# icdm-adteam/MoCoPCI

Hardware: AMD Instinct MI355X
Metric: interpolated frames/sec (higher is better)
Workload: dtype f32 (fused MLP layers: fp32 products as 6 bf16-MFMA partials of an exact 3-way split, fp32 accumulate; index paths exact f32)

## Files before the change

mocopci_amd/csrc/fusion.hip:

```cpp
#include <stdlib.h>

#include "common.h"
#include "mfma_split.h"

namespace {

typedef float f32x16 __attribute__((ext_vector_type(16)));

constexpr int C1 = 64, C2 = 64, NB = 64;
constexpr int WAVES = 4;


__device__ __forceinline__ int chan_of(int r, int h) { return (r & 3) + 8 * (r >> 2) + 4 * h; }

__device__ __forceinline__ float wave_sum(float v) {
#pragma unroll
    for (int o = 32; o > 0; o >>= 1) v += __shfl_xor(v, o);
    return v;
}
__device__ __forceinline__ float wave_max(float v) {
#pragma unroll
    for (int o = 32; o > 0; o >>= 1) v = fmaxf(v, __shfl_xor(v, o));
    return v;
}

#ifdef MCP_AB
constexpr int OFF_W1 = 0, OFF_W2 = 256, OFF_W3 = OFF_W2 + 4096, OFF_B1 = OFF_W3 + 8192, OFF_B2 = OFF_B1 + 64,
              OFF_B3 = OFF_B2 + 64, LDS_FLOATS = OFF_B3 + 128;
__global__ __launch_bounds__(64 * WAVES, 2) void fusion_kernel(long long total, int n, const float *__restrict__ p1,
                                                            const float *__restrict__ p2, const int *__restrict__ idx, const int *__restrict__ idx2,
                                                            const float *__restrict__ w1, const float *__restrict__ b1,
                                                            const float *__restrict__ w2, const float *__restrict__ b2,
                                                            const float *__restrict__ w3, const float *__restrict__ b3,
                                                            float *__restrict__ out) {
    __shared__ __attribute__((aligned(16))) float lds[LDS_FLOATS];
    const int tid = threadIdx.x;
    for (int e = tid; e < 256; e += 64 * WAVES) {
        const int lane = e & 63, s = (e >> 6) & 1, t = e >> 7;
        lds[OFF_W1 + e] = w1[(32 * t + (lane & 31)) * 4 + 2 * s + (lane >> 5)];
    }
    for (int e = tid; e < 4096; e += 64 * WAVES) {
        const int j = e & 3, lane = (e >> 2) & 63, q = (e >> 8) & 7, t = e >> 11;
        const int s = 4 * q + j, tin = s >> 4, r = s & 15;
        lds[OFF_W2 + e] = w2[(32 * t + (lane & 31)) * C1 + 32 * tin + chan_of(r, lane >> 5)];
    }
    for (int e = tid; e < 8192; e += 64 * WAVES) {
        const int j = e & 3, lane = (e >> 2) & 63, q = (e >> 8) & 7, t = e >> 11;
        const int s = 4 * q + j, tin = s >> 4, r = s & 15;
        lds[OFF_W3 + e] = w3[(32 * t + (lane & 31)) * C2 + 32 * tin + chan_of(r, lane >> 5)];
    }
    for (int e = tid; e < 64; e += 64 * WAVES) {
        const int r = e & 15, h = (e >> 4) & 1, t = e >> 5;
        lds[OFF_B1 + e] = b1[32 * t + chan_of(r, h)];
        lds[OFF_B2 + e] = b2[32 * t + chan_of(r, h)];
    }
    for (int e = tid; e < 128; e += 64 * WAVES) {
        const int r = e & 15, h = (e >> 4) & 1, t = e >> 5;
        lds[OFF_B3 + e] = b3[32 * t + chan_of(r, h)];
    }
    __syncthreads();

    const int lane = tid & 63, wave = tid >> 6, h = lane >> 5, col = lane & 31;
    const float4 *w2q = reinterpret_cast<const float4 *>(lds + OFF_W2);
    const float4 *w3q = reinterpret_cast<const float4 *>(lds + OFF_W3);

    const McpUnits units = mcp_units_by_xcd(total, WAVES);
    for (long long p = units.first + wave; p < units.limit; p += units.stride) {
        const long long bb = mcp_div(p, n, mcp_fits32(total));
        const float cx = p1[p * 3 + 0], cy = p1[p * 3 + 1], cz = p1[p * 3 + 2];
        float score[2], nbx[2], nby[2], nbz[2];
#pragma unroll
        for (int ct = 0; ct < 2; ++ct) {
            const int id = idx2 ? (ct ? idx2 : idx)[p * 32 + col] : idx[p * NB + 32 * ct + col];
            const float *q = p2 + ((long long)bb * n + id) * 3;
            const float x = q[0], y = q[1], z = q[2];
            nbx[ct] = x; nby[ct] = y; nbz[ct] = z;
            const float rx = x - cx, ry = y - cy, rz = z - cz;
            const float dist = sqrtf((rx * rx + ry * ry) + rz * rz);
            const float in0 = h ? ry : rx, in1 = h ? dist : rz;
            f32x16 a1[2];
#pragma unroll
            for (int t = 0; t < 2; ++t) {
                f32x16 acc;
#pragma unroll
                for (int r = 0; r < 16; ++r) acc[r] = lds[OFF_B1 + (t * 2 + h) * 16 + r];
                acc = __builtin_amdgcn_mfma_f32_32x32x2f32(lds[OFF_W1 + (t * 2 + 0) * 64 + lane], in0, acc, 0, 0, 0);
                acc = __builtin_amdgcn_mfma_f32_32x32x2f32(lds[OFF_W1 + (t * 2 + 1) * 64 + lane], in1, acc, 0, 0, 0);
#pragma unroll
                for (int r = 0; r < 16; ++r) acc[r] = fmaxf(acc[r], 0.f);
                a1[t] = acc;
            }
            f32x16 a2[2];
#pragma unroll
            for (int t = 0; t < 2; ++t) {
                f32x16 acc;
#pragma unroll
                for (int r = 0; r < 16; ++r) acc[r] = lds[OFF_B2 + (t * 2 + h) * 16 + r];
#pragma unroll
                for (int q4 = 0; q4 < 8; ++q4) {
                    const float4 w = w2q[(t * 8 + q4) * 64 + lane];
                    const int tin = q4 >> 2, r0 = (q4 & 3) * 4;
                    acc = __builtin_amdgcn_mfma_f32_32x32x2f32(w.x, a1[tin][r0 + 0], acc, 0, 0, 0);
                    acc = __builtin_amdgcn_mfma_f32_32x32x2f32(w.y, a1[tin][r0 + 1], acc, 0, 0, 0);
                    acc = __builtin_amdgcn_mfma_f32_32x32x2f32(w.z, a1[tin][r0 + 2], acc, 0, 0, 0);
                    acc = __builtin_amdgcn_mfma_f32_32x32x2f32(w.w, a1[tin][r0 + 3], acc, 0, 0, 0);
                }
#pragma unroll
                for (int r = 0; r < 16; ++r) acc[r] = fmaxf(acc[r], 0.f);
                a2[t] = acc;
            }
            float m = 0.f;
#pragma unroll 1
            for (int t = 0; t < 4; ++t) {
                f32x16 acc;
#pragma unroll
                for (int r = 0; r < 16; ++r) acc[r] = lds[OFF_B3 + (t * 2 + h) * 16 + r];
#pragma unroll
                for (int q4 = 0; q4 < 8; ++q4) {
                    const float4 w = w3q[(t * 8 + q4) * 64 + lane];
                    const int tin = q4 >> 2, r0 = (q4 & 3) * 4;
                    acc = __builtin_amdgcn_mfma_f32_32x32x2f32(w.x, a2[tin][r0 + 0], acc, 0, 0, 0);
                    acc = __builtin_amdgcn_mfma_f32_32x32x2f32(w.y, a2[tin][r0 + 1], acc, 0, 0, 0);
                    acc = __builtin_amdgcn_mfma_f32_32x32x2f32(w.z, a2[tin][r0 + 2], acc, 0, 0, 0);
                    acc = __builtin_amdgcn_mfma_f32_32x32x2f32(w.w, a2[tin][r0 + 3], acc, 0, 0, 0);
                }
#pragma unroll
                for (int r = 0; r < 16; ++r) m = fmaxf(m, acc[r]);
            }
            score[ct] = fmaxf(m, __shfl_xor(m, 32));
        }
        const float mx = wave_max(fmaxf(score[0], score[1]));
        const float e0 = expf(score[0] - mx), e1 = expf(score[1] - mx);
        const float den = wave_sum(e0 + e1);
        const float sx = wave_sum(e0 * nbx[0] + e1 * nbx[1]);
        const float sy = wave_sum(e0 * nby[0] + e1 * nby[1]);
        const float sz = wave_sum(e0 * nbz[0] + e1 * nbz[1]);
        if (lane == 0) {
            out[p * 3 + 0] = sx / den;
            out[p * 3 + 1] = sy / den;
            out[p * 3 + 2] = sz / den;
        }
    }
}
#endif


constexpr int SP_W1 = 0, SP_B1 = 256, SP_B2 = SP_B1 + 64, SP_B3 = SP_B2 + 64, SP_F32_FLOATS = SP_B3 + 128;
constexpr int SP_W2_U4 = 2 * 4 * 3 * 64, SP_W3_U4 = 4 * 4 * 3 * 64;
constexpr size_t SP_LDS_BYTES = SP_F32_FLOATS * 4 + (size_t)(SP_W2_U4 + SP_W3_U4) * 16;

__global__ __launch_bounds__(64 * WAVES, 2) void fusion_split_kernel(long long total, int n, const float *__restrict__ p1,
                                                                  const float *__restrict__ p2, const int *__restrict__ idx, const int *__restrict__ idx2,
                                                                  const float *__restrict__ w1, const float *__restrict__ b1,
                                                                  const float *__restrict__ w2, const float *__restrict__ b2,
                                                                  const float *__restrict__ w3, const float *__restrict__ b3,
                                                                  float *__restrict__ out) {
    extern __shared__ __attribute__((aligned(16))) float lds[];
    uint4 *w2s = reinterpret_cast<uint4 *>(lds + SP_F32_FLOATS);
    uint4 *w3s = w2s + SP_W2_U4;
    const int tid = threadIdx.x;
    for (int e = tid; e < 256; e += 64 * WAVES) {
        const int lane = e & 63, s = (e >> 6) & 1, t = e >> 7;
        lds[SP_W1 + e] = w1[(32 * t + (lane & 31)) * 4 + 2 * s + (lane >> 5)];
    }
    mcp_split_weights(w2s, w2, C1, 2, tid, 64 * WAVES);
    mcp_split_weights(w3s, w3, C2, 4, tid, 64 * WAVES);
    for (int e = tid; e < 64; e += 64 * WAVES) {
        const int r = e & 15, h = (e >> 4) & 1, t = e >> 5;
        lds[SP_B1 + e] = b1[32 * t + chan_of(r, h)];
        lds[SP_B2 + e] = b2[32 * t + chan_of(r, h)];
    }
    for (int e = tid; e < 128; e += 64 * WAVES) {
        const int r = e & 15, h = (e >> 4) & 1, t = e >> 5;
        lds[SP_B3 + e] = b3[32 * t + chan_of(r, h)];
    }
    __syncthreads();

    const int lane = tid & 63, wave = tid >> 6, h = lane >> 5, col = lane & 31;
    const McpUnits units = mcp_units_by_xcd(total, WAVES);
    for (long long p = units.first + wave; p < units.limit; p += units.stride) {
        const long long bb = mcp_div(p, n, mcp_fits32(total));
        const float cx = p1[p * 3 + 0], cy = p1[p * 3 + 1], cz = p1[p * 3 + 2];
        float score[2], nbx[2], nby[2], nbz[2];
#pragma unroll
        for (int ct = 0; ct < 2; ++ct) {
            const int id = idx2 ? (ct ? idx2 : idx)[p * 32 + col] : idx[p * NB + 32 * ct + col];
            const float *q = p2 + ((long long)bb * n + id) * 3;
            const float x = q[0], y = q[1], z = q[2];
            nbx[ct] = x; nby[ct] = y; nbz[ct] = z;
            const float rx = x - cx, ry = y - cy, rz = z - cz;
            const float dist = sqrtf((rx * rx + ry * ry) + rz * rz);
            const float in0 = h ? ry : rx, in1 = h ? dist : rz;
            McpSplit3 x1[4];
#pragma unroll
            for (int t = 0; t < 2; ++t) {
                f32x16 acc;
#pragma unroll
                for (int r = 0; r < 16; ++r) acc[r] = lds[SP_B1 + (t * 2 + h) * 16 + r];
                acc = __builtin_amdgcn_mfma_f32_32x32x2f32(lds[SP_W1 + (t * 2 + 0) * 64 + lane], in0, acc, 0, 0, 0);
                acc = __builtin_amdgcn_mfma_f32_32x32x2f32(lds[SP_W1 + (t * 2 + 1) * 64 + lane], in1, acc, 0, 0, 0);
#pragma unroll
                for (int r = 0; r < 16; ++r) acc[r] = fmaxf(acc[r], 0.f);
                x1[2 * t + 0] = mcp_split_kstep(acc, 0);
                x1[2 * t + 1] = mcp_split_kstep(acc, 1);
            }
            McpSplit3 x2[4];
#pragma unroll
            for (int t = 0; t < 2; ++t) {
                f32x16 acc;
#pragma unroll
                for (int r = 0; r < 16; ++r) acc[r] = lds[SP_B2 + (t * 2 + h) * 16 + r];
                acc = mcp_tile_split<4>(w2s + (size_t)t * 4 * 3 * 64 + lane, x1, acc);
#pragma unroll
                for (int r = 0; r < 16; ++r) acc[r] = fmaxf(acc[r], 0.f);
                x2[2 * t + 0] = mcp_split_kstep(acc, 0);
                x2[2 * t + 1] = mcp_split_kstep(acc, 1);
            }
            float m = 0.f;
#pragma unroll 1
            for (int t = 0; t < 4; ++t) {
                f32x16 acc;
#pragma unroll
                for (int r = 0; r < 16; ++r) acc[r] = lds[SP_B3 + (t * 2 + h) * 16 + r];
                acc = mcp_tile_split<4>(w3s + (size_t)t * 4 * 3 * 64 + lane, x2, acc);
#pragma unroll
                for (int r = 0; r < 16; ++r) m = fmaxf(m, acc[r]);
            }
            score[ct] = fmaxf(m, __shfl_xor(m, 32));
        }
        const float mx = wave_max(fmaxf(score[0], score[1]));
        const float e0 = expf(score[0] - mx), e1 = expf(score[1] - mx);
        const float den = wave_sum(e0 + e1);
        const float sx = wave_sum(e0 * nbx[0] + e1 * nbx[1]);
        const float sy = wave_sum(e0 * nby[0] + e1 * nby[1]);
        const float sz = wave_sum(e0 * nbz[0] + e1 * nbz[1]);
        if (lane == 0) {
            out[p * 3 + 0] = sx / den;
            out[p * 3 + 1] = sy / den;
            out[p * 3 + 2] = sz / den;
        }
    }
}

}

MCP_EXPORT int mcp_fusion(int b, int n, int nb, const float *p1, const float *p2, const int *idx, const int *idx2, const float *w1,
                          const float *b1, const float *w2, const float *b2, const float *w3, const float *b3, float *out,
                          mcp_stream_t stream) {
    MCP_CHECK_ARGS(b > 0 && n > 0 && p1 && p2 && idx && w1 && b1 && w2 && b2 && w3 && b3 && out);
    if (nb != NB) return MCP_ERR_UNSUPPORTED;
    hipStream_t s = (hipStream_t)stream;
    const long long total = (long long)b * n;
    long long grid_cap = 4096;
#ifdef MCP_AB
    static const long long env_cap = [] { const char *v = getenv("MCP_FUSION_GRID"); return (long long)(v && *v ? atoi(v) : 0); }();
    if (env_cap >= 1) grid_cap = env_cap;
    static const bool f32_mfma = [] { const char *v = getenv("MCP_FUSION_F32_MFMA"); return v && *v == '1'; }();
#endif
    const unsigned grid = (unsigned)min((total + WAVES - 1) / WAVES, grid_cap);
    mcp_prof_begin(MCP_KERNEL_FUSION, s);
#ifdef MCP_AB
    if (f32_mfma) {
        hipLaunchKernelGGL(fusion_kernel, dim3(grid), dim3(64 * WAVES), 0, s, total, n, p1, p2, idx, idx2, w1, b1, w2, b2, w3, b3, out);
        mcp_prof_end(MCP_KERNEL_FUSION, s);
        return mcp_launch_status();
    }
#endif
    static McpPerDeviceOnce attr_once;
    if (attr_once.need()) {
        { const hipError_t attr_e_ = hipFuncSetAttribute(reinterpret_cast<const void *>(fusion_split_kernel), hipFuncAttributeMaxDynamicSharedMemorySize, 160 * 1024); if (attr_e_ != hipSuccess) return (int)attr_e_; }
        attr_once.done();
    }
    hipLaunchKernelGGL(fusion_split_kernel, dim3(grid), dim3(64 * WAVES), SP_LDS_BYTES, s, total, n, p1, p2, idx, idx2, w1, b1, w2, b2, w3, b3, out);
    mcp_prof_end(MCP_KERNEL_FUSION, s);
    return mcp_launch_status();
}
```

mocopci_amd/csrc/mfma_split.h:

```cpp
#pragma once
#include "common.h"

#ifndef MCP_SPLIT_SCHED_MASK
#define MCP_SPLIT_SCHED_MASK 0x0000
#endif

typedef float mcp_f32x16 __attribute__((ext_vector_type(16)));
typedef __bf16 mcp_bf16x8 __attribute__((ext_vector_type(8)));

__device__ __forceinline__ int mcp_chan_of(int r, int h) { return (r & 3) + 8 * (r >> 2) + 4 * h; }
__device__ __forceinline__ uint32_t mcp_top16(float x) { return __float_as_uint(x) & 0xFFFF0000u; }
__device__ __forceinline__ uint32_t mcp_pack_hi(float even, float odd) {
    return __builtin_amdgcn_perm(__float_as_uint(odd), __float_as_uint(even), 0x07060302u);
}

struct McpSplit3 {
    uint4 p1, p2, p3;
};
__device__ __forceinline__ McpSplit3 mcp_split8(const float *v) {
    float r1[8], r2[8];
#pragma unroll
    for (int i = 0; i < 8; ++i) {
        r1[i] = v[i] - __uint_as_float(mcp_top16(v[i]));
        r2[i] = r1[i] - __uint_as_float(mcp_top16(r1[i]));
    }
    McpSplit3 o;
#ifdef MCP_SPLIT_DIAG_NOSPLIT
    o.p1 = make_uint4(mcp_pack_hi(v[0], v[1]), mcp_pack_hi(v[2], v[3]), mcp_pack_hi(v[4], v[5]), mcp_pack_hi(v[6], v[7]));
    o.p2 = o.p1; o.p3 = o.p1;
    return o;
#endif
    o.p1 = make_uint4(mcp_pack_hi(v[0], v[1]), mcp_pack_hi(v[2], v[3]), mcp_pack_hi(v[4], v[5]), mcp_pack_hi(v[6], v[7]));
    o.p2 = make_uint4(mcp_pack_hi(r1[0], r1[1]), mcp_pack_hi(r1[2], r1[3]), mcp_pack_hi(r1[4], r1[5]), mcp_pack_hi(r1[6], r1[7]));
    o.p3 = make_uint4(mcp_pack_hi(r2[0], r2[1]), mcp_pack_hi(r2[2], r2[3]), mcp_pack_hi(r2[4], r2[5]), mcp_pack_hi(r2[6], r2[7]));
    return o;
}
__device__ __forceinline__ McpSplit3 mcp_split_kstep(const mcp_f32x16 &a, int s) {
    float v[8];
#pragma unroll
    for (int i = 0; i < 8; ++i) v[i] = a[8 * s + i];
    return mcp_split8(v);
}
__device__ __forceinline__ mcp_f32x16 mcp_mfma_bf16(uint4 a, uint4 b, mcp_f32x16 c) {
    return __builtin_amdgcn_mfma_f32_32x32x16_bf16(__builtin_bit_cast(mcp_bf16x8, a), __builtin_bit_cast(mcp_bf16x8, b), c, 0, 0, 0);
}
__device__ __forceinline__ mcp_f32x16 mcp_mfma_split(const uint4 *w, const McpSplit3 &x, mcp_f32x16 acc) {
    const uint4 w1 = w[0], w2 = w[64], w3 = w[128];
    acc = mcp_mfma_bf16(w3, x.p1, acc);
    acc = mcp_mfma_bf16(w1, x.p3, acc);
    acc = mcp_mfma_bf16(w2, x.p2, acc);
    acc = mcp_mfma_bf16(w2, x.p1, acc);
    acc = mcp_mfma_bf16(w1, x.p2, acc);
    acc = mcp_mfma_bf16(w1, x.p1, acc);
    return acc;
}
template <int KSTEPS>
__device__ __forceinline__ mcp_f32x16 mcp_tile_split(const uint4 *ws, const McpSplit3 *xs, mcp_f32x16 acc) {
    uint4 w1 = ws[0], w2 = ws[64], w3 = ws[128];
#pragma unroll
    for (int s = 0; s < KSTEPS; ++s) {
        uint4 n1 = w1, n2 = w2, n3 = w3;
#ifndef MCP_SPLIT_DIAG_NOLOAD
        if (s + 1 < KSTEPS) {
            const uint4 *nx = ws + (size_t)(s + 1) * 3 * 64;
            n1 = nx[0]; n2 = nx[64]; n3 = nx[128];
        }
#endif
        acc = mcp_mfma_bf16(w3, xs[s].p1, acc);
        acc = mcp_mfma_bf16(w1, xs[s].p3, acc);
        acc = mcp_mfma_bf16(w2, xs[s].p2, acc);
        acc = mcp_mfma_bf16(w2, xs[s].p1, acc);
        acc = mcp_mfma_bf16(w1, xs[s].p2, acc);
        acc = mcp_mfma_bf16(w1, xs[s].p1, acc);
        __builtin_amdgcn_sched_barrier(MCP_SPLIT_SCHED_MASK);
        w1 = n1; w2 = n2; w3 = n3;
    }
    return acc;
}

__device__ __forceinline__ void mcp_split_weights(uint4 *dst, const float *__restrict__ w, int cin, int out_tiles, int first, int stride) {
    const int ksteps = cin / 16;
    for (int e = first; e < out_tiles * ksteps * 64; e += stride) {
        const int lane = e & 63, s = (e >> 6) % ksteps, t = (e >> 6) / ksteps;
        float v[8];
#pragma unroll
        for (int i = 0; i < 8; ++i) v[i] = w[(size_t)(32 * t + (lane & 31)) * cin + 32 * (s >> 1) + mcp_chan_of(8 * (s & 1) + i, lane >> 5)];
        const McpSplit3 sp = mcp_split8(v);
        uint4 *o = dst + (size_t)(t * ksteps + s) * 3 * 64 + lane;
        o[0] = sp.p1;
        o[64] = sp.p2;
        o[128] = sp.p3;
    }
}
```

Measured before the change: 3569.

## Interleave both neighbor tiles through MLP layers and overlap split work with MFMA

```diff
diff --git a/mocopci_amd/csrc/fusion.hip b/mocopci_amd/csrc/fusion.hip
--- a/mocopci_amd/csrc/fusion.hip
+++ b/mocopci_amd/csrc/fusion.hip
@@ -9,6 +9,9 @@
 
 constexpr int C1 = 64, C2 = 64, NB = 64;
 constexpr int WAVES = 4;
+#ifndef FUSION_FILL
+#define FUSION_FILL 5
+#endif
 
 
 __device__ __forceinline__ int chan_of(int r, int h) { return (r & 3) + 8 * (r >> 2) + 4 * h; }
@@ -182,6 +185,7 @@
         const long long bb = mcp_div(p, n, mcp_fits32(total));
         const float cx = p1[p * 3 + 0], cy = p1[p * 3 + 1], cz = p1[p * 3 + 2];
         float score[2], nbx[2], nby[2], nbz[2];
+        McpSplit3 x1[2][4];
 #pragma unroll
         for (int ct = 0; ct < 2; ++ct) {
             const int id = idx2 ? (ct ? idx2 : idx)[p * 32 + col] : idx[p * NB + 32 * ct + col];
@@ -191,7 +195,6 @@
             const float rx = x - cx, ry = y - cy, rz = z - cz;
             const float dist = sqrtf((rx * rx + ry * ry) + rz * rz);
             const float in0 = h ? ry : rx, in1 = h ? dist : rz;
-            McpSplit3 x1[4];
 #pragma unroll
             for (int t = 0; t < 2; ++t) {
                 f32x16 acc;
@@ -201,33 +204,60 @@
                 acc = __builtin_amdgcn_mfma_f32_32x32x2f32(lds[SP_W1 + (t * 2 + 1) * 64 + lane], in1, acc, 0, 0, 0);
 #pragma unroll
                 for (int r = 0; r < 16; ++r) acc[r] = fmaxf(acc[r], 0.f);
-                x1[2 * t + 0] = mcp_split_kstep(acc, 0);
-                x1[2 * t + 1] = mcp_split_kstep(acc, 1);
-            }
-            McpSplit3 x2[4];
-#pragma unroll
-            for (int t = 0; t < 2; ++t) {
-                f32x16 acc;
-#pragma unroll
-                for (int r = 0; r < 16; ++r) acc[r] = lds[SP_B2 + (t * 2 + h) * 16 + r];
-                acc = mcp_tile_split<4>(w2s + (size_t)t * 4 * 3 * 64 + lane, x1, acc);
-#pragma unroll
-                for (int r = 0; r < 16; ++r) acc[r] = fmaxf(acc[r], 0.f);
-                x2[2 * t + 0] = mcp_split_kstep(acc, 0);
-                x2[2 * t + 1] = mcp_split_kstep(acc, 1);
-            }
-            float m = 0.f;
+                x1[ct][2 * t + 0] = mcp_split_kstep(acc, 0);
+                x1[ct][2 * t + 1] = mcp_split_kstep(acc, 1);
+            }
+        }
+        McpSplit3 x2[2][4];
+        f32x16 a2[2], c2[2];
+#pragma unroll
+        for (int r = 0; r < 16; ++r) a2[0][r] = a2[1][r] = lds[SP_B2 + (0 * 2 + h) * 16 + r];
+        mcp_tile_split2<4>(w2s + lane, x1[0], x1[1], a2[0], a2[1]);
+#pragma unroll
+        for (int r = 0; r < 16; ++r) c2[0][r] = c2[1][r] = lds[SP_B2 + (1 * 2 + h) * 16 + r];
+        mcp_tile_split2<4, FUSION_FILL>(w2s + (size_t)4 * 3 * 64 + lane, x1[0], x1[1], c2[0], c2[1], [&](int s) {
+            const int ct = s >> 1, part = s & 1;
+            float v[8];
+#pragma unroll
+            for (int i = 0; i < 8; ++i) v[i] = fmaxf(a2[ct][8 * part + i], 0.f);
+            x2[ct][part] = mcp_split8(v);
+        });
+        float m[2] = {0.f, 0.f};
+        f32x16 a3[2];
+#pragma unroll
+        for (int r = 0; r < 16; ++r) a3[0][r] = a3[1][r] = lds[SP_B3 + (0 * 2 + h) * 16 + r];
+        mcp_tile_split2<4, FUSION_FILL>(w3s + lane, x2[0], x2[1], a3[0], a3[1], [&](int s) {
+            if (s < 2) {
+#pragma unroll
+                for (int ct = 0; ct < 2; ++ct) {
+                    float v[8];
+#pragma unroll
+                    for (int i = 0; i < 8; ++i) v[i] = fmaxf(c2[ct][8 * s + i], 0.f);
+                    x2[ct][2 + s] = mcp_split8(v);
+                }
+            }
+        });
 #pragma unroll 1
-            for (int t = 0; t < 4; ++t) {
-                f32x16 acc;
-#pragma unroll
-                for (int r = 0; r < 16; ++r) acc[r] = lds[SP_B3 + (t * 2 + h) * 16 + r];
-                acc = mcp_tile_split<4>(w3s + (size_t)t * 4 * 3 * 64 + lane, x2, acc);
-#pragma unroll
-                for (int r = 0; r < 16; ++r) m = fmaxf(m, acc[r]);
-            }
-            score[ct] = fmaxf(m, __shfl_xor(m, 32));
-        }
+        for (int t = 1; t < 4; ++t) {
+            f32x16 n3[2];
+#pragma unroll
+            for (int r = 0; r < 16; ++r) n3[0][r] = n3[1][r] = lds[SP_B3 + (t * 2 + h) * 16 + r];
+            mcp_tile_split2<4, FUSION_FILL>(w3s + (size_t)t * 4 * 3 * 64 + lane, x2[0], x2[1], n3[0], n3[1], [&](int s) {
+                if (s == 0) {
+#pragma unroll
+                    for (int ct = 0; ct < 2; ++ct)
+#pragma unroll
+                        for (int r = 0; r < 16; ++r) m[ct] = fmaxf(m[ct], a3[ct][r]);
+                }
+            });
+            a3[0] = n3[0];
+            a3[1] = n3[1];
+        }
+#pragma unroll
+        for (int ct = 0; ct < 2; ++ct)
+#pragma unroll
+            for (int r = 0; r < 16; ++r) m[ct] = fmaxf(m[ct], a3[ct][r]);
+        for (int ct = 0; ct < 2; ++ct) score[ct] = fmaxf(m[ct], __shfl_xor(m[ct], 32));
         const float mx = wave_max(fmaxf(score[0], score[1]));
         const float e0 = expf(score[0] - mx), e1 = expf(score[1] - mx);
         const float den = wave_sum(e0 + e1);
diff --git a/mocopci_amd/csrc/mfma_split.h b/mocopci_amd/csrc/mfma_split.h
--- a/mocopci_amd/csrc/mfma_split.h
+++ b/mocopci_amd/csrc/mfma_split.h
@@ -77,6 +77,44 @@
     }
     return acc;
 }
+struct McpNoFill {
+    __device__ __forceinline__ void operator()(int) const {}
+};
+template <int KSTEPS, int FILL_PER_GAP = 0, class Fill = McpNoFill>
+__device__ __forceinline__ void mcp_tile_split2(const uint4 *ws, const McpSplit3 *xa, const McpSplit3 *xb, mcp_f32x16 &acc_a,
+                                                mcp_f32x16 &acc_b, Fill fill = Fill()) {
+    uint4 w1 = ws[0], w2 = ws[64], w3 = ws[128];
+#pragma unroll
+    for (int s = 0; s < KSTEPS; ++s) {
+        uint4 n1 = w1, n2 = w2, n3 = w3;
+        if (s + 1 < KSTEPS) {
+            const uint4 *nx = ws + (size_t)(s + 1) * 3 * 64;
+            n1 = nx[0]; n2 = nx[64]; n3 = nx[128];
+        }
+        fill(s);
+        acc_a = mcp_mfma_bf16(w3, xa[s].p1, acc_a);
+        acc_b = mcp_mfma_bf16(w3, xb[s].p1, acc_b);
+        acc_a = mcp_mfma_bf16(w1, xa[s].p3, acc_a);
+        acc_b = mcp_mfma_bf16(w1, xb[s].p3, acc_b);
+        acc_a = mcp_mfma_bf16(w2, xa[s].p2, acc_a);
+        acc_b = mcp_mfma_bf16(w2, xb[s].p2, acc_b);
+        acc_a = mcp_mfma_bf16(w2, xa[s].p1, acc_a);
+        acc_b = mcp_mfma_bf16(w2, xb[s].p1, acc_b);
+        acc_a = mcp_mfma_bf16(w1, xa[s].p2, acc_a);
+        acc_b = mcp_mfma_bf16(w1, xb[s].p2, acc_b);
+        acc_a = mcp_mfma_bf16(w1, xa[s].p1, acc_a);
+        acc_b = mcp_mfma_bf16(w1, xb[s].p1, acc_b);
+        if (FILL_PER_GAP > 0) {
+#pragma unroll
+            for (int g = 0; g < 12; ++g) {
+                __builtin_amdgcn_sched_group_barrier(0x008, 1, 0);
+                __builtin_amdgcn_sched_group_barrier(0x002, FILL_PER_GAP, 0);
+            }
+        }
+        __builtin_amdgcn_sched_barrier(MCP_SPLIT_SCHED_MASK);
+        w1 = n1; w2 = n2; w3 = n3;
+    }
+}
 
 __device__ __forceinline__ void mcp_split_weights(uint4 *dst, const float *__restrict__ w, int cin, int out_tiles, int first, int stride) {
     const int ksteps = cin / 16;
```

Result: faster. 3656, median of 6 (+2.4%).

## Software-pipeline MLP regions across neighbor tiles with interleaved MFMA/VALU scheduling

Applied to the files above, without the earlier changes.

```diff
diff --git a/mocopci_amd/csrc/fusion.hip b/mocopci_amd/csrc/fusion.hip
--- a/mocopci_amd/csrc/fusion.hip
+++ b/mocopci_amd/csrc/fusion.hip
@@ -177,68 +177,114 @@
     __syncthreads();
 
     const int lane = tid & 63, wave = tid >> 6, h = lane >> 5, col = lane & 31;
+    const bool fits = mcp_fits32(total);
+    auto id_of = [&](long long q, int ct) -> int {
+        return idx2 ? (ct ? idx2 : idx)[q * 32 + col] : idx[q * NB + 32 * ct + col];
+    };
+    auto nb_of = [&](long long q, int id) -> const float * { return p2 + ((long long)mcp_div(q, n, fits) * n + id) * 3; };
+    auto front_a = [&](f32x16 *a1, float x, float y, float z, float cx, float cy, float cz) {
+        const float rx = x - cx, ry = y - cy, rz = z - cz;
+        const float dist = sqrtf((rx * rx + ry * ry) + rz * rz);
+        const float in0 = h ? ry : rx, in1 = h ? dist : rz;
+#pragma unroll
+        for (int t = 0; t < 2; ++t) {
+            f32x16 acc;
+#pragma unroll
+            for (int r = 0; r < 16; ++r) acc[r] = lds[SP_B1 + (t * 2 + h) * 16 + r];
+            acc = __builtin_amdgcn_mfma_f32_32x32x2f32(lds[SP_W1 + (t * 2 + 0) * 64 + lane], in0, acc, 0, 0, 0);
+            acc = __builtin_amdgcn_mfma_f32_32x32x2f32(lds[SP_W1 + (t * 2 + 1) * 64 + lane], in1, acc, 0, 0, 0);
+            a1[t] = acc;
+        }
+    };
+    auto relu_split = [&](McpSplit3 *x, f32x16 acc) {
+#pragma unroll
+        for (int r = 0; r < 16; ++r) acc[r] = fmaxf(acc[r], 0.f);
+        x[0] = mcp_split_kstep(acc, 0);
+        x[1] = mcp_split_kstep(acc, 1);
+        mcp_pin(x[0]);
+        mcp_pin(x[1]);
+    };
+    auto layer2 = [&](const McpSplit3 *x1, int t) -> f32x16 {
+        f32x16 acc;
+#pragma unroll
+        for (int r = 0; r < 16; ++r) acc[r] = lds[SP_B2 + (t * 2 + h) * 16 + r];
+        return mcp_tile_split<4, false>(w2s + (size_t)t * 4 * 3 * 64 + lane, x1, acc);
+    };
+    auto layer3 = [&](const McpSplit3 *x2, int t) -> f32x16 {
+        f32x16 acc;
+#pragma unroll
+        for (int r = 0; r < 16; ++r) acc[r] = lds[SP_B3 + (t * 2 + h) * 16 + r];
+        return mcp_tile_split<4, false>(w3s + (size_t)t * 4 * 3 * 64 + lane, x2, acc);
+    };
+    auto chan_max = [&](float m, const f32x16 &acc) {
+#pragma unroll
+        for (int r = 0; r < 16; ++r) m = fmaxf(m, acc[r]);
+        return m;
+    };
+    auto region = [&](const McpSplit3 *x2, McpSplit3 *x2n, float x, float y, float z, float cx, float cy, float cz) -> float {
+        f32x16 a1[2], c0, c1, c2, c3, l2a, l2b;
+        McpSplit3 x1[4];
+        float m = 0.f;
+        mcp_interleave<52, 5>([&] { front_a(a1, x, y, z, cx, cy, cz); c0 = layer3(x2, 0); c1 = layer3(x2, 1); },
+                              [&] { relu_split(x1, a1[0]); relu_split(x1 + 2, a1[1]); m = chan_max(m, c0); });
+        mcp_interleave<24, 1>([&] { l2a = layer2(x1, 0); }, [&] { m = chan_max(m, c1); });
+        mcp_interleave<48, 3>([&] { c2 = layer3(x2, 2); l2b = layer2(x1, 1); }, [&] { relu_split(x2n, l2a); });
+        mcp_interleave<24, 5>([&] { c3 = layer3(x2, 3); }, [&] { relu_split(x2n + 2, l2b); m = chan_max(m, c2); });
+        m = chan_max(m, c3);
+        return fmaxf(m, __shfl_xor(m, 32));
+    };
+    auto front = [&](McpSplit3 *x2, float x, float y, float z, float cx, float cy, float cz) {
+        f32x16 a1[2];
+        McpSplit3 x1[4];
+        front_a(a1, x, y, z, cx, cy, cz);
+        relu_split(x1, a1[0]);
+        relu_split(x1 + 2, a1[1]);
+        relu_split(x2, layer2(x1, 0));
+        relu_split(x2 + 2, layer2(x1, 1));
+    };
+
     const McpUnits units = mcp_units_by_xcd(total, WAVES);
-    for (long long p = units.first + wave; p < units.limit; p += units.stride) {
-        const long long bb = mcp_div(p, n, mcp_fits32(total));
-        const float cx = p1[p * 3 + 0], cy = p1[p * 3 + 1], cz = p1[p * 3 + 2];
-        float score[2], nbx[2], nby[2], nbz[2];
-#pragma unroll
-        for (int ct = 0; ct < 2; ++ct) {
-            const int id = idx2 ? (ct ? idx2 : idx)[p * 32 + col] : idx[p * NB + 32 * ct + col];
-            const float *q = p2 + ((long long)bb * n + id) * 3;
-            const float x = q[0], y = q[1], z = q[2];
-            nbx[ct] = x; nby[ct] = y; nbz[ct] = z;
-            const float rx = x - cx, ry = y - cy, rz = z - cz;
-            const float dist = sqrtf((rx * rx + ry * ry) + rz * rz);
-            const float in0 = h ? ry : rx, in1 = h ? dist : rz;
-            McpSplit3 x1[4];
-#pragma unroll
-            for (int t = 0; t < 2; ++t) {
-                f32x16 acc;
-#pragma unroll
-                for (int r = 0; r < 16; ++r) acc[r] = lds[SP_B1 + (t * 2 + h) * 16 + r];
-                acc = __builtin_amdgcn_mfma_f32_32x32x2f32(lds[SP_W1 + (t * 2 + 0) * 64 + lane], in0, acc, 0, 0, 0);
-                acc = __builtin_amdgcn_mfma_f32_32x32x2f32(lds[SP_W1 + (t * 2 + 1) * 64 + lane], in1, acc, 0, 0, 0);
-#pragma unroll
-                for (int r = 0; r < 16; ++r) acc[r] = fmaxf(acc[r], 0.f);
-                x1[2 * t + 0] = mcp_split_kstep(acc, 0);
-                x1[2 * t + 1] = mcp_split_kstep(acc, 1);
-            }
-            McpSplit3 x2[4];
-#pragma unroll
-            for (int t = 0; t < 2; ++t) {
-                f32x16 acc;
-#pragma unroll
-                for (int r = 0; r < 16; ++r) acc[r] = lds[SP_B2 + (t * 2 + h) * 16 + r];
-                acc = mcp_tile_split<4>(w2s + (size_t)t * 4 * 3 * 64 + lane, x1, acc);
-#pragma unroll
-                for (int r = 0; r < 16; ++r) acc[r] = fmaxf(acc[r], 0.f);
-                x2[2 * t + 0] = mcp_split_kstep(acc, 0);
-                x2[2 * t + 1] = mcp_split_kstep(acc, 1);
-            }
-            float m = 0.f;
-#pragma unroll 1
-            for (int t = 0; t < 4; ++t) {
-                f32x16 acc;
-#pragma unroll
-                for (int r = 0; r < 16; ++r) acc[r] = lds[SP_B3 + (t * 2 + h) * 16 + r];
-                acc = mcp_tile_split<4>(w3s + (size_t)t * 4 * 3 * 64 + lane, x2, acc);
-#pragma unroll
-                for (int r = 0; r < 16; ++r) m = fmaxf(m, acc[r]);
-            }
-            score[ct] = fmaxf(m, __shfl_xor(m, 32));
-        }
-        const float mx = wave_max(fmaxf(score[0], score[1]));
-        const float e0 = expf(score[0] - mx), e1 = expf(score[1] - mx);
+    long long p = units.first + wave;
+    if (p >= units.limit) return;
+    auto next_of = [&](long long q) { return q + units.stride < units.limit ? q + units.stride : q; };
+    float cx = p1[p * 3 + 0], cy = p1[p * 3 + 1], cz = p1[p * 3 + 2];
+    McpSplit3 x2a[4], x2b[4];
+    float nx0, ny0, nz0, nx1, ny1, nz1;
+    {
+        const float *q = nb_of(p, id_of(p, 0));
+        nx0 = q[0]; ny0 = q[1]; nz0 = q[2];
+        q = nb_of(p, id_of(p, 1));
+        nx1 = q[0]; ny1 = q[1]; nz1 = q[2];
+    }
+    int id_n0 = id_of(next_of(p), 0);
+    front(x2a, nx0, ny0, nz0, cx, cy, cz);
+    for (;;) {
+        const long long pn = next_of(p);
+        const float cxn = p1[pn * 3 + 0], cyn = p1[pn * 3 + 1], czn = p1[pn * 3 + 2];
+        const float *qa = nb_of(pn, id_n0);
+        const float nx0n = qa[0], ny0n = qa[1], nz0n = qa[2];
+        const int id_n1 = id_of(pn, 1);
+        const float m0 = region(x2a, x2b, nx1, ny1, nz1, cx, cy, cz);
+        const float *qb = nb_of(pn, id_n1);
+        const float nx1n = qb[0], ny1n = qb[1], nz1n = qb[2];
+        id_n0 = id_of(next_of(pn), 0);
+        const float m1 = region(x2b, x2a, nx0n, ny0n, nz0n, cxn, cyn, czn);
+        const float mx = wave_max(fmaxf(m0, m1));
+        const float e0 = expf(m0 - mx), e1 = expf(m1 - mx);
         const float den = wave_sum(e0 + e1);
-        const float sx = wave_sum(e0 * nbx[0] + e1 * nbx[1]);
-        const float sy = wave_sum(e0 * nby[0] + e1 * nby[1]);
-        const float sz = wave_sum(e0 * nbz[0] + e1 * nbz[1]);
+        const float sx = wave_sum(e0 * nx0 + e1 * nx1);
+        const float sy = wave_sum(e0 * ny0 + e1 * ny1);
+        const float sz = wave_sum(e0 * nz0 + e1 * nz1);
         if (lane == 0) {
             out[p * 3 + 0] = sx / den;
             out[p * 3 + 1] = sy / den;
             out[p * 3 + 2] = sz / den;
         }
+        if (pn == p) break;
+        p = pn;
+        cx = cxn; cy = cyn; cz = czn;
+        nx0 = nx0n; ny0 = ny0n; nz0 = nz0n;
+        nx1 = nx1n; ny1 = ny1n; nz1 = nz1n;
     }
 }
 
diff --git a/mocopci_amd/csrc/mfma_split.h b/mocopci_amd/csrc/mfma_split.h
--- a/mocopci_amd/csrc/mfma_split.h
+++ b/mocopci_amd/csrc/mfma_split.h
@@ -54,7 +54,7 @@
     acc = mcp_mfma_bf16(w1, x.p1, acc);
     return acc;
 }
-template <int KSTEPS>
+template <int KSTEPS, bool FENCE = true>
 __device__ __forceinline__ mcp_f32x16 mcp_tile_split(const uint4 *ws, const McpSplit3 *xs, mcp_f32x16 acc) {
     uint4 w1 = ws[0], w2 = ws[64], w3 = ws[128];
 #pragma unroll
@@ -72,10 +72,25 @@
         acc = mcp_mfma_bf16(w2, xs[s].p1, acc);
         acc = mcp_mfma_bf16(w1, xs[s].p2, acc);
         acc = mcp_mfma_bf16(w1, xs[s].p1, acc);
-        __builtin_amdgcn_sched_barrier(MCP_SPLIT_SCHED_MASK);
+        if (FENCE) __builtin_amdgcn_sched_barrier(MCP_SPLIT_SCHED_MASK);
         w1 = n1; w2 = n2; w3 = n3;
     }
     return acc;
+}
+
+__device__ __forceinline__ void mcp_pin(uint4 &v) { asm volatile("" : "+v"(v.x), "+v"(v.y), "+v"(v.z), "+v"(v.w)); }
+__device__ __forceinline__ void mcp_pin(McpSplit3 &x) { mcp_pin(x.p1); mcp_pin(x.p2); mcp_pin(x.p3); }
+template <int NMFMA, int NVALU, class Matrix, class Vector>
+__device__ __forceinline__ void mcp_interleave(Matrix &&matrix, Vector &&vector) {
+    __builtin_amdgcn_sched_barrier(0);
+    matrix();
+    vector();
+#pragma unroll
+    for (int i = 0; i < NMFMA; ++i) {
+        __builtin_amdgcn_sched_group_barrier(0x008, 1, 0);
+        __builtin_amdgcn_sched_group_barrier(0x002, NVALU, 0);
+    }
+    __builtin_amdgcn_sched_barrier(0);
 }
 
 __device__ __forceinline__ void mcp_split_weights(uint4 *dst, const float *__restrict__ w, int cin, int out_tiles, int first, int stride) {
```

After: 3615 before, 3638 after (median of 6 runs). No clear change (+0.6%).
